# ChengZhang-98/lqer

Measured on AMD Instinct MI355X. Metric: W4A8+rank-r Linear GEMM TFLOPS-equiv, higher is better.
Workload: dtype bf16; 1 GPU; LqerLinear 4096x4096 rank32 W4A8-MXINT16 M=2048 (BASELINE configs[1]); rank=32, formats=x MXINT8/16, W MXINT4/16, A_out,B_out as x, y fp16, weights=one Linear

## Files before the change

lqer_amd/csrc/act16_fused.hip:

```cpp
#include "common.h"

namespace lqer {
namespace a16f {

constexpr int ROWS = 8, WAVES = 8, SLAB = 512, PITCH = 1040;

__host__ inline size_t lds_bytes(int rp) { return (size_t)WAVES * ROWS * PITCH + (size_t)WAVES * ROWS * rp * sizeof(float); }

typedef __attribute__((ext_vector_type(8))) __bf16 bf16v8;

#ifdef LQER_CLOCKPROBE
__device__ unsigned long long* g_a16_stamp_buf = nullptr;
#define A16_STAMP(i) asm volatile("s_memtime %0\n\ts_waitcnt lgkmcnt(0)" : "=s"(cp[i])::"memory")
#else
#define A16_STAMP(i)
#endif

template <int DT, int RT>
__global__ __launch_bounds__(512) void k_act16_fused(const void* __restrict__ x, int64_t M, int64_t K, int64_t ld, QP qx, bf16_t* __restrict__ xq,
                                                      int64_t Kp, const bf16_t* __restrict__ a_frag, QP qa, int L_aout, bf16_t* __restrict__ xaq) {
  constexpr int RP = 16 * RT;
  constexpr int HB = RT == 8 ? 2 : (RT == 4 ? 4 : 8);
  constexpr int NPART = 16 / HB;
  extern __shared__ __attribute__((aligned(16))) unsigned char smem[];
  const int lane = threadIdx.x & 63;
  const int wave = __builtin_amdgcn_readfirstlane(threadIdx.x >> 6);
  unsigned char* const wb = smem + (size_t)wave * ROWS * PITCH;
  float* const red = (float*)(smem + (size_t)WAVES * ROWS * PITCH);
  const int64_t m0 = (int64_t)blockIdx.x * ROWS;
  const int nslab = (int)((Kp + SLAB - 1) / SLAB);
  const int g = lane >> 4;
  const unsigned char* const tok = wb + (lane & 7) * PITCH + 16 * g;
  const u32x4* const fr = (const u32x4*)a_frag + lane;
  f32x4 acc[RT];
#pragma unroll
  for (int t = 0; t < RT; ++t) acc[t] = (f32x4){0.f, 0.f, 0.f, 0.f};
#ifdef LQER_CLOCKPROBE
  unsigned long long cp[8] = {0, 0, 0, 0, 0, 0, 0, 0};
  A16_STAMP(0);
#endif

  for (int s = wave; s < nslab; s += WAVES) {
    const int64_t k0 = (int64_t)s * SLAB + 8 * lane;
    const bool in_img = k0 < Kp, in_x = k0 < K;
    u32x4 raw[ROWS];
#pragma unroll
    for (int r = 0; r < ROWS; ++r)
      raw[r] = (in_x && m0 + r < M) ? *(const u32x4*)((const bf16_t*)x + (m0 + r) * ld + k0) : (u32x4){0, 0, 0, 0};
    const int st0 = s * (SLAB / 32), nst = (int)(Kp / 32);
    u32x4 fa[HB][RT], fb[HB][RT];
    auto load_part = [&](u32x4 (&f)[HB][RT], int part) {
#pragma unroll
      for (int i = 0; i < HB; ++i)
#pragma unroll
        for (int t = 0; t < RT; ++t) {
          const int st = st0 + part * HB + i;
          f[i][t] = fr[((int64_t)(st < nst ? st : 0) * RT + t) * 64];
        }
    };
    if (s == wave) A16_STAMP(1);
#pragma unroll
    for (int r = 0; r < ROWS; ++r) {
      if (r == 1 && s == wave) A16_STAMP(2);
      if (r == 2) {
        asm volatile("" ::: "memory");
        load_part(fa, 0);
        asm volatile("" ::: "memory");
      }
      if (r == 5) {
        asm volatile("" ::: "memory");
        load_part(fb, 1);
        asm volatile("" ::: "memory");
      }
      float v[8];
      const uint32_t wd[4] = {raw[r][0], raw[r][1], raw[r][2], raw[r][3]};
#pragma unroll
      for (int j = 0; j < 4; ++j) {
        if constexpr (DT == LQER_F16) {
          typedef __attribute__((ext_vector_type(2))) _Float16 h2;
          const h2 h = __builtin_bit_cast(h2, wd[j]);
          v[2 * j] = (float)h[0], v[2 * j + 1] = (float)h[1];
        } else {
          v[2 * j] = __uint_as_float(wd[j] << 16), v[2 * j + 1] = __uint_as_float(wd[j] & 0xffff0000u);
        }
      }
      float amax = 0.f;
#pragma unroll
      for (int i = 0; i < 8; ++i) amax = fmaxf(amax, fabsf(v[i]));
      amax = fmaxf(amax, __shfl_xor(amax, 1, 64));
      uint32_t w[4] = {0, 0, 0, 0};
      if (amax > 0.f) {
        const int e = block_exponent_u(amax, qx);
        if (mxint16_fast_ok(e, qx)) {
          mxint16_bf16_fast<DT != LQER_F16, 8>(v, e, qx, w);
        } else {
#pragma unroll
          for (int i = 0; i < 4; ++i) {
            const uint32_t lo = exact_bf16_bits(ldexpf(mxint_mantissa(v[2 * i], e, qx), e - qx.mbits));
            const uint32_t hi = exact_bf16_bits(ldexpf(mxint_mantissa(v[2 * i + 1], e, qx), e - qx.mbits));
            w[i] = lo | (hi << 16);
          }
        }
      }
      const u32x4 wv = {w[0], w[1], w[2], w[3]};
      if (in_img) *(u32x4*)(xq + (m0 + r) * Kp + k0) = wv;
      *(u32x4*)(wb + r * PITCH + 16 * lane) = wv;
    }
    if (s == wave) A16_STAMP(3);
    __builtin_amdgcn_fence(__ATOMIC_RELEASE, "wavefront");
    __builtin_amdgcn_wave_barrier();
    __builtin_amdgcn_fence(__ATOMIC_ACQUIRE, "wavefront");
    auto half = [&](const u32x4 (&f)[HB][RT], int t0) {
      u32x4 tk[HB];
#pragma unroll
      for (int i = 0; i < HB; ++i) tk[i] = *(const u32x4*)(tok + 64 * (t0 + i));
#pragma unroll
      for (int i = 0; i < HB; ++i)
#pragma unroll
        for (int t = 0; t < RT; ++t)
          acc[t] = __builtin_amdgcn_mfma_f32_16x16x32_bf16(__builtin_bit_cast(bf16v8, tk[i]), __builtin_bit_cast(bf16v8, f[i][t]), acc[t], 0, 0, 0);
    };
#pragma unroll
    for (int pp = 0; pp < NPART; pp += 2) {
      half(fa, pp * HB);
      if (pp + 2 < NPART) load_part(fa, pp + 2);
      half(fb, (pp + 1) * HB);
      if (pp + 3 < NPART) load_part(fb, pp + 3);
    }
    __builtin_amdgcn_fence(__ATOMIC_RELEASE, "wavefront");
    __builtin_amdgcn_wave_barrier();
#ifdef LQER_CLOCKPROBE
    if (s == wave) {
      asm volatile("" ::"v"(acc[0]));
      A16_STAMP(4);
    }
#endif
  }
  if (g < 2) {
#pragma unroll
    for (int t = 0; t < RT; ++t)
#pragma unroll
      for (int j = 0; j < 4; ++j) red[(wave * ROWS + 4 * g + j) * RP + 16 * t + (lane & 15)] = acc[t][j];
  }
  __syncthreads();
#ifdef LQER_CLOCKPROBE
  A16_STAMP(5);
  if (g_a16_stamp_buf && lane == 0) {
    unsigned long long* o = g_a16_stamp_buf + ((size_t)blockIdx.x * WAVES + wave) * 8;
    for (int i = 1; i < 6; ++i) o[i] = cp[i] - cp[0];
    unsigned long long rt;
    asm volatile("s_memrealtime %0\n\ts_waitcnt lgkmcnt(0)" : "=s"(rt)::"memory");
    o[0] = cp[0], o[6] = rt;
  }
#endif
  const int tid = threadIdx.x;
  const bool live = tid < ROWS * RP / 4;
  const int r = tid / (RP / 4), c4 = tid - r * (RP / 4);
  float4 sum = make_float4(0.f, 0.f, 0.f, 0.f);
  if (live) {
#pragma unroll
    for (int w = 0; w < WAVES; ++w) {
      const float4 v = *(const float4*)(red + (w * ROWS + r) * RP + 4 * c4);
      sum.x += v.x, sum.y += v.y, sum.z += v.z, sum.w += v.w;
    }
  }
  if (tid >= 64 * ((ROWS * RP / 4 + 63) / 64)) return;
  float bmax = fmaxf(fmaxf(fabsf(sum.x), fabsf(sum.y)), fmaxf(fabsf(sum.z), fabsf(sum.w)));
  const int G = L_aout / 4;
  for (int d = 1; d < G; d <<= 1) bmax = fmaxf(bmax, __shfl_xor(bmax, d, 64));
  if (!live || m0 + r >= M) return;
  const bool anyb = bmax > 0.f;
  const int eb = anyb ? block_exponent(bmax, qa) : 0;
  const float v[4] = {sum.x, sum.y, sum.z, sum.w};
  uint32_t w2[2];
#pragma unroll
  for (int i = 0; i < 2; ++i) {
    const float m0v = anyb ? mxint_mantissa(v[2 * i], eb, qa) : 0.f;
    const float m1v = anyb ? mxint_mantissa(v[2 * i + 1], eb, qa) : 0.f;
    w2[i] = exact_bf16_bits(ldexpf(m0v, eb - qa.mbits)) | (exact_bf16_bits(ldexpf(m1v, eb - qa.mbits)) << 16);
  }
  *(uint2*)(xaq + ((m0 + r) * RP + 4 * c4)) = make_uint2(w2[0], w2[1]);
}

__global__ __launch_bounds__(256) void k_a_b16(const bf16_t* __restrict__ limb0, int64_t Kp, int rp, bf16_t* __restrict__ out) {
  const int RT = rp / 16;
  const int64_t n_img = (int64_t)rp * Kp / 8, total = 2 * n_img;
  for (int64_t idx = (int64_t)blockIdx.x * 256 + threadIdx.x; idx < total; idx += (int64_t)gridDim.x * 256) {
    if (idx < n_img) {
      ((u32x4*)out)[idx] = ((const u32x4*)limb0)[idx];
    } else {
      const int64_t f = idx - n_img;
      const int lane = (int)(f & 63);
      const int64_t blk = f >> 6;
      const int t = (int)(blk % RT);
      const int64_t s = blk / RT;
      ((u32x4*)out)[idx] = *(const u32x4*)(limb0 + (int64_t)(16 * t + (lane & 15)) * Kp + 32 * s + 8 * (lane >> 4));
    }
  }
}

}

#ifdef LQER_CLOCKPROBE
extern "C" int lqer_debug_set_a16_stamp_buffer(void* p) { return (int)hipMemcpyToSymbol(HIP_SYMBOL(a16f::g_a16_stamp_buf), &p, sizeof(p)); }
#endif

size_t a_b16_image_bytes(int64_t K, int64_t r) { return (size_t)2 * lqer_padded_r(r) * lqer_padded_k(K) * sizeof(bf16_t); }

int a_b16_prepare_dispatch(const void* a_t_limbs, int64_t K, int64_t r, void* out, hipStream_t st) {
  const int64_t rp = lqer_padded_r(r), Kp = lqer_padded_k(K);
  if (rp % 16 != 0 || Kp % 32 != 0) {
    set_error("a_b16_prepare: padded rank %d / padded K %d", (int)rp, (int)Kp);
    return LQER_E_UNSUPPORTED;
  }
  const int64_t total = 2 * rp * Kp / 8;
  a16f::k_a_b16<<<(unsigned)((total + 255) / 256 < 4096 ? (total + 255) / 256 : 4096), 256, 0, st>>>((const bf16_t*)a_t_limbs, Kp, (int)rp, (bf16_t*)out);
  return check_launch("a_b16_prepare");
}

int act16_fused_dispatch(const void* x, int dtype, int64_t M, int64_t K, int64_t ldx, const QP& qx, bf16_t* xq, const void* a_b16, int64_t r,
                         const QP& qa, bf16_t* xaq, int tuning, hipStream_t st) {
  if (tuning & LQER_TUNE_ACT16_SPLIT) return LQER_E_UNSUPPORTED;
  const int64_t rp = lqer_padded_r(r), Kp = lqer_padded_k(K);
  if (dtype == LQER_F32 || !a_b16 || !xaq || !xq || r <= 0 || M <= 0) return LQER_E_UNSUPPORTED;
  if (!(rp == 16 || rp == 32 || rp == 64)) return LQER_E_UNSUPPORTED;
  if (qx.kind != LQER_Q_MXINT || qx.block != 16 || qx.mbits > 8) return LQER_E_UNSUPPORTED;
  if (((uintptr_t)x % 16) != 0 || ((ldx * 2) % 16) != 0 || K % 16 != 0) return LQER_E_UNSUPPORTED;
  if (qa.kind != LQER_Q_MXINT || qa.mbits > 8) return LQER_E_UNSUPPORTED;
  const int L = (qa.block <= 0 || qa.block >= rp) ? (int)rp : qa.block;
  const int G = L / 4;
  if (rp % L != 0 || L % 4 != 0 || (G & (G - 1)) != 0 || G > 64) return LQER_E_UNSUPPORTED;
  if (!(tuning & LQER_TUNE_ACT16_FUSED) && (M > LQER_ACT8_FUSED_MAX_M || M < LQER_ACT8_FUSED_MIN_M)) return LQER_E_UNSUPPORTED;
  const bf16_t* const a_frag = (const bf16_t*)a_b16 + rp * Kp;
  const unsigned grid = (unsigned)((M + a16f::ROWS - 1) / a16f::ROWS);
  const int lds = (int)a16f::lds_bytes((int)rp);
#define A16F_LAUNCH(DTv, RTv)                                                                                              \
  do {                                                                                                                     \
    static LdsLimitOnce once;                                                                                              \
    once.set((const void*)a16f::k_act16_fused<DTv, RTv>, 160 * 1024);                                                       \
    a16f::k_act16_fused<DTv, RTv><<<grid, 512, lds, st>>>(x, M, K, ldx, qx, xq, Kp, a_frag, qa, L, xaq);                     \
  } while (0)
#define A16F_DT(DTv)                     \
  switch (rp / 16) {                     \
    case 1: A16F_LAUNCH(DTv, 1); break;  \
    case 2: A16F_LAUNCH(DTv, 2); break;  \
    default: A16F_LAUNCH(DTv, 4); break; \
  }
  if (dtype == LQER_F16) {
    A16F_DT(LQER_F16)
  } else {
    A16F_DT(LQER_BF16)
  }
#undef A16F_DT
#undef A16F_LAUNCH
  return check_launch("quantize_act_xa (fused block-16 route)");
}

}
```

Before: 1057 TFLOP/s-equiv.

## Split fused act16 quantize+XA kernel across 16 waves sharing slabs

```diff
diff --git a/lqer_amd/csrc/act16_fused.hip b/lqer_amd/csrc/act16_fused.hip
--- a/lqer_amd/csrc/act16_fused.hip
+++ b/lqer_amd/csrc/act16_fused.hip
@@ -3,9 +3,9 @@
 namespace lqer {
 namespace a16f {
 
-constexpr int ROWS = 8, WAVES = 8, SLAB = 512, PITCH = 1040;
-
-__host__ inline size_t lds_bytes(int rp) { return (size_t)WAVES * ROWS * PITCH + (size_t)WAVES * ROWS * rp * sizeof(float); }
+constexpr int ROWS = 8, SLABS = 8, WAVES = 16, WROWS = 4, SLAB = 512, PITCH = 1040;
+
+__host__ inline size_t lds_bytes(int rp) { return (size_t)SLABS * ROWS * PITCH + (size_t)SLABS * ROWS * rp * sizeof(float); }
 
 typedef __attribute__((ext_vector_type(8))) __bf16 bf16v8;
 
@@ -16,141 +16,217 @@
 #define A16_STAMP(i)
 #endif
 
+__device__ __forceinline__ float pair_max(float v) {
+  return fmaxf(v, __int_as_float(__builtin_amdgcn_update_dpp(0, __float_as_int(v), 0xB1, 0xf, 0xf, true)));
+}
+
+template <int DT>
+__device__ __forceinline__ void row_values(const u32x4& raw, float (&v)[8]) {
+#pragma unroll
+  for (int i = 0; i < 4; ++i) {
+    const uint32_t wd = raw[i];
+    if constexpr (DT == LQER_F16) {
+      typedef __attribute__((ext_vector_type(2))) _Float16 h2;
+      const h2 hh = __builtin_bit_cast(h2, wd);
+      v[2 * i] = (float)hh[0], v[2 * i + 1] = (float)hh[1];
+    } else {
+      v[2 * i] = __uint_as_float(wd << 16), v[2 * i + 1] = __uint_as_float(wd & 0xffff0000u);
+    }
+  }
+}
+
+template <int DT>
+__device__ __forceinline__ u32x4 row_bits(const float (&v)[8]) {
+  u32x4 r;
+#pragma unroll
+  for (int i = 0; i < 4; ++i) {
+    if constexpr (DT == LQER_F16) r[i] = __builtin_bit_cast(uint32_t, __builtin_amdgcn_cvt_pkrtz(v[2 * i], v[2 * i + 1]));
+    else r[i] = (__float_as_uint(v[2 * i]) >> 16) | (__float_as_uint(v[2 * i + 1]) & 0xffff0000u);
+  }
+  return r;
+}
+
+template <int DT>
+__device__ __forceinline__ void quantize_rows_slow(unsigned char* rows, const QP& qx, bf16_t* img, int64_t Kp, bool in_img) {
+#pragma unroll 1
+  for (int j = 0; j < WROWS; ++j) {
+    float v[8];
+    row_values<DT>(*(const u32x4*)(rows + j * PITCH), v);
+    float amax = 0.f;
+#pragma unroll
+    for (int i = 0; i < 8; ++i) amax = fmaxf(amax, fabsf(v[i]));
+    amax = pair_max(amax);
+    uint32_t w[4] = {0, 0, 0, 0};
+    if (amax > 0.f) {
+      const int e = block_exponent_u(amax, qx);
+      if (mxint16_fast_ok(e, qx)) {
+        mxint16_bf16_fast<DT != LQER_F16, 8>(v, e, qx, w);
+      } else {
+#pragma unroll
+        for (int i = 0; i < 4; ++i) {
+          const uint32_t lo = exact_bf16_bits(ldexpf(mxint_mantissa(v[2 * i], e, qx), e - qx.mbits));
+          const uint32_t hi = exact_bf16_bits(ldexpf(mxint_mantissa(v[2 * i + 1], e, qx), e - qx.mbits));
+          w[i] = lo | (hi << 16);
+        }
+      }
+    }
+    const u32x4 wv = {w[0], w[1], w[2], w[3]};
+    if (in_img) *(u32x4*)(img + j * Kp) = wv;
+    *(u32x4*)(rows + j * PITCH) = wv;
+  }
+}
+
 template <int DT, int RT>
-__global__ __launch_bounds__(512) void k_act16_fused(const void* __restrict__ x, int64_t M, int64_t K, int64_t ld, QP qx, bf16_t* __restrict__ xq,
-                                                      int64_t Kp, const bf16_t* __restrict__ a_frag, QP qa, int L_aout, bf16_t* __restrict__ xaq) {
+__global__ __launch_bounds__(1024) void k_act16_fused(const void* __restrict__ x, int64_t M, int64_t K, int64_t ld, QP qx, bf16_t* __restrict__ xq,
+                                                       int64_t Kp, const bf16_t* __restrict__ a_frag, QP qa, int L_aout, bf16_t* __restrict__ xaq) {
   constexpr int RP = 16 * RT;
-  constexpr int HB = RT == 8 ? 2 : (RT == 4 ? 4 : 8);
+  constexpr int TW = RT >= 2 ? RT / 2 : 1;
+  constexpr int HB = TW == 2 ? 4 : 8;
   constexpr int NPART = 16 / HB;
   extern __shared__ __attribute__((aligned(16))) unsigned char smem[];
+  asm volatile("" ::"s"(x), "s"(M), "s"(K), "s"(ld), "s"(xq), "s"(Kp), "s"(a_frag), "s"(xaq), "s"(L_aout), "s"(qx.mbits), "s"(qx.emin), "s"(qx.emax),
+               "s"(qx.mmax), "s"(qx.mneg), "s"(qx.eps), "s"(qx.tiny), "s"(qa.mbits), "s"(qa.emin), "s"(qa.emax), "s"(qa.mmax), "s"(qa.mneg), "s"(qa.eps),
+               "s"(qa.tiny));
   const int lane = threadIdx.x & 63;
   const int wave = __builtin_amdgcn_readfirstlane(threadIdx.x >> 6);
-  unsigned char* const wb = smem + (size_t)wave * ROWS * PITCH;
-  float* const red = (float*)(smem + (size_t)WAVES * ROWS * PITCH);
+  const int sl = wave & (SLABS - 1), h = wave >> 3;
+  unsigned char* const sb = smem + (size_t)sl * ROWS * PITCH;
+  float* const red = (float*)(smem + (size_t)SLABS * ROWS * PITCH);
   const int64_t m0 = (int64_t)blockIdx.x * ROWS;
   const int nslab = (int)((Kp + SLAB - 1) / SLAB);
+  const int ntrip = (nslab + SLABS - 1) / SLABS;
   const int g = lane >> 4;
-  const unsigned char* const tok = wb + (lane & 7) * PITCH + 16 * g;
+  const unsigned char* const tok = sb + (lane & 7) * PITCH + 16 * g;
   const u32x4* const fr = (const u32x4*)a_frag + lane;
-  f32x4 acc[RT];
-#pragma unroll
-  for (int t = 0; t < RT; ++t) acc[t] = (f32x4){0.f, 0.f, 0.f, 0.f};
+  const int t0w = RT >= 2 ? h * TW : 0;
+  const int64_t row0 = m0 + WROWS * h;
+  const int nrow = M - row0 >= WROWS ? WROWS : (int)(M - row0);
+  const int xstep = (int)(ld * 2), qstep = (int)(Kp * 2);
+  const auto xr = __builtin_amdgcn_make_buffer_rsrc((void*)((const unsigned char*)x + row0 * ld * 2), 0, nrow > 0 ? (nrow - 1) * xstep + (int)(K * 2) : 0,
+                                                    0x00020000);
+  const auto qr = __builtin_amdgcn_make_buffer_rsrc((void*)((unsigned char*)xq + row0 * Kp * 2), 0, WROWS * qstep, 0x00020000);
+  f32x4 acc[TW];
+#pragma unroll
+  for (int t = 0; t < TW; ++t) acc[t] = (f32x4){0.f, 0.f, 0.f, 0.f};
 #ifdef LQER_CLOCKPROBE
   unsigned long long cp[8] = {0, 0, 0, 0, 0, 0, 0, 0};
   A16_STAMP(0);
 #endif
 
-  for (int s = wave; s < nslab; s += WAVES) {
-    const int64_t k0 = (int64_t)s * SLAB + 8 * lane;
-    const bool in_img = k0 < Kp, in_x = k0 < K;
-    u32x4 raw[ROWS];
-#pragma unroll
-    for (int r = 0; r < ROWS; ++r)
-      raw[r] = (in_x && m0 + r < M) ? *(const u32x4*)((const bf16_t*)x + (m0 + r) * ld + k0) : (u32x4){0, 0, 0, 0};
+  for (int it = 0; it < ntrip; ++it) {
+    const int s = it * SLABS + sl;
+    const bool live_slab = s < nslab;
     const int st0 = s * (SLAB / 32), nst = (int)(Kp / 32);
-    u32x4 fa[HB][RT], fb[HB][RT];
-    auto load_part = [&](u32x4 (&f)[HB][RT], int part) {
+    u32x4 fa[HB][TW], fb[HB][TW];
+    auto load_part = [&](u32x4 (&f)[HB][TW], int part) {
 #pragma unroll
       for (int i = 0; i < HB; ++i)
 #pragma unroll
-        for (int t = 0; t < RT; ++t) {
+        for (int t = 0; t < TW; ++t) {
           const int st = st0 + part * HB + i;
-          f[i][t] = fr[((int64_t)(st < nst ? st : 0) * RT + t) * 64];
+          f[i][t] = fr[((int64_t)(st < nst ? st : 0) * RT + t0w + t) * 64];
         }
     };
-    if (s == wave) A16_STAMP(1);
-#pragma unroll
-    for (int r = 0; r < ROWS; ++r) {
-      if (r == 1 && s == wave) A16_STAMP(2);
-      if (r == 2) {
-        asm volatile("" ::: "memory");
-        load_part(fa, 0);
-        asm volatile("" ::: "memory");
-      }
-      if (r == 5) {
-        asm volatile("" ::: "memory");
-        load_part(fb, 1);
-        asm volatile("" ::: "memory");
-      }
-      float v[8];
-      const uint32_t wd[4] = {raw[r][0], raw[r][1], raw[r][2], raw[r][3]};
-#pragma unroll
-      for (int j = 0; j < 4; ++j) {
-        if constexpr (DT == LQER_F16) {
-          typedef __attribute__((ext_vector_type(2))) _Float16 h2;
-          const h2 h = __builtin_bit_cast(h2, wd[j]);
-          v[2 * j] = (float)h[0], v[2 * j + 1] = (float)h[1];
-        } else {
-          v[2 * j] = __uint_as_float(wd[j] << 16), v[2 * j + 1] = __uint_as_float(wd[j] & 0xffff0000u);
+    if (live_slab) {
+      const int kb = s * (SLAB * 2) + 16 * lane;
+      const int xoff = kb < (int)(K * 2) ? kb : -1 - WROWS * xstep, qoff = kb < qstep ? kb : -1 - WROWS * qstep;
+      u32x4 raw[WROWS];
+#pragma unroll
+      for (int j = 0; j < WROWS; ++j) raw[j] = __builtin_amdgcn_raw_buffer_load_b128(xr, xoff + j * xstep, 0, 0);
+      load_part(fa, 0);
+      if (it == 0) A16_STAMP(1);
+      float v[WROWS][8], amax[WROWS];
+      int e[WROWS];
+      bool near = false;
+#pragma unroll
+      for (int j = 0; j < WROWS; ++j) {
+        row_values<DT>(raw[j], v[j]);
+        float a = 0.f;
+#pragma unroll
+        for (int i = 0; i < 8; ++i) a = fmaxf(a, fabsf(v[j][i]));
+        amax[j] = a = pair_max(a);
+        const uint32_t bits = __float_as_uint(a);
+        const int eb = (int)((bits >> 23) & 0xff) - 126;
+        e[j] = eb < qx.emin ? qx.emin : (eb > qx.emax ? qx.emax : eb);
+        near |= (bits & 0x7fffffu) <= 22u && a > 0.f;
+      }
+      if (__builtin_amdgcn_ballot_w64(near) != 0) {
+#pragma unroll
+        for (int j = 0; j < WROWS; ++j) e[j] = block_exponent(amax[j], qx);
+      }
+      bool slow = false;
+#pragma unroll
+      for (int j = 0; j < WROWS; ++j) slow |= amax[j] > 0.f && !mxint16_fast_ok(e[j], qx);
+      if (it == 0) A16_STAMP(2);
+      if (__builtin_amdgcn_ballot_w64(slow) == 0) {
+        uint32_t w[WROWS][4];
+#pragma unroll
+        for (int j = 0; j < WROWS; ++j) {
+          mxint16_bf16_fast<DT != LQER_F16, 8>(v[j], e[j], qx, w[j]);
+          uint32_t keep = amax[j] > 0.f ? 0xffffffffu : 0u;
+          asm("" : "+v"(keep));
+#pragma unroll
+          for (int i = 0; i < 4; ++i) w[j][i] &= keep;
         }
-      }
-      float amax = 0.f;
-#pragma unroll
-      for (int i = 0; i < 8; ++i) amax = fmaxf(amax, fabsf(v[i]));
-      amax = fmaxf(amax, __shfl_xor(amax, 1, 64));
-      uint32_t w[4] = {0, 0, 0, 0};
-      if (amax > 0.f) {
-        const int e = block_exponent_u(amax, qx);
-        if (mxint16_fast_ok(e, qx)) {
-          mxint16_bf16_fast<DT != LQER_F16, 8>(v, e, qx, w);
-        } else {
-#pragma unroll
-          for (int i = 0; i < 4; ++i) {
-            const uint32_t lo = exact_bf16_bits(ldexpf(mxint_mantissa(v[2 * i], e, qx), e - qx.mbits));
-            const uint32_t hi = exact_bf16_bits(ldexpf(mxint_mantissa(v[2 * i + 1], e, qx), e - qx.mbits));
-            w[i] = lo | (hi << 16);
-          }
+#pragma unroll
+        for (int j = 0; j < WROWS; ++j) {
+          const u32x4 wv = {w[j][0], w[j][1], w[j][2], w[j][3]};
+          __builtin_amdgcn_raw_buffer_store_b128(wv, qr, qoff + j * qstep, 0, 0);
+          *(u32x4*)(sb + (WROWS * h + j) * PITCH + 16 * lane) = wv;
         }
-      }
-      const u32x4 wv = {w[0], w[1], w[2], w[3]};
-      if (in_img) *(u32x4*)(xq + (m0 + r) * Kp + k0) = wv;
-      *(u32x4*)(wb + r * PITCH + 16 * lane) = wv;
-    }
-    if (s == wave) A16_STAMP(3);
-    __builtin_amdgcn_fence(__ATOMIC_RELEASE, "wavefront");
-    __builtin_amdgcn_wave_barrier();
-    __builtin_amdgcn_fence(__ATOMIC_ACQUIRE, "wavefront");
-    auto half = [&](const u32x4 (&f)[HB][RT], int t0) {
-      u32x4 tk[HB];
-#pragma unroll
-      for (int i = 0; i < HB; ++i) tk[i] = *(const u32x4*)(tok + 64 * (t0 + i));
-#pragma unroll
-      for (int i = 0; i < HB; ++i)
-#pragma unroll
-        for (int t = 0; t < RT; ++t)
-          acc[t] = __builtin_amdgcn_mfma_f32_16x16x32_bf16(__builtin_bit_cast(bf16v8, tk[i]), __builtin_bit_cast(bf16v8, f[i][t]), acc[t], 0, 0, 0);
-    };
-#pragma unroll
-    for (int pp = 0; pp < NPART; pp += 2) {
-      half(fa, pp * HB);
-      if (pp + 2 < NPART) load_part(fa, pp + 2);
-      half(fb, (pp + 1) * HB);
-      if (pp + 3 < NPART) load_part(fb, pp + 3);
-    }
-    __builtin_amdgcn_fence(__ATOMIC_RELEASE, "wavefront");
-    __builtin_amdgcn_wave_barrier();
-#ifdef LQER_CLOCKPROBE
-    if (s == wave) {
+      } else {
+#pragma unroll
+        for (int j = 0; j < WROWS; ++j) *(u32x4*)(sb + (WROWS * h + j) * PITCH + 16 * lane) = row_bits<DT>(v[j]);
+        quantize_rows_slow<DT>(sb + WROWS * h * PITCH + 16 * lane, qx, xq + (m0 + WROWS * h) * Kp + (int64_t)s * SLAB + 8 * lane, Kp,
+                               (int64_t)s * SLAB + 8 * lane < Kp);
+      }
+      load_part(fb, 1);
+      if (it == 0) A16_STAMP(3);
+    }
+    __syncthreads();
+    if (it == 0) A16_STAMP(4);
+    if (live_slab) {
+      auto half = [&](const u32x4 (&f)[HB][TW], int t0) {
+        u32x4 tk[HB];
+#pragma unroll
+        for (int i = 0; i < HB; ++i) tk[i] = *(const u32x4*)(tok + 64 * (t0 + i));
+#pragma unroll
+        for (int i = 0; i < HB; ++i)
+#pragma unroll
+          for (int t = 0; t < TW; ++t)
+            acc[t] = __builtin_amdgcn_mfma_f32_16x16x32_bf16(__builtin_bit_cast(bf16v8, tk[i]), __builtin_bit_cast(bf16v8, f[i][t]), acc[t], 0, 0, 0);
+      };
+#pragma unroll
+      for (int pp = 0; pp < NPART; pp += 2) {
+        half(fa, pp * HB);
+        if (pp + 2 < NPART) load_part(fa, pp + 2);
+        half(fb, (pp + 1) * HB);
+        if (pp + 3 < NPART) load_part(fb, pp + 3);
+      }
+    }
+#ifdef LQER_CLOCKPROBE
+    if (it == 0) {
       asm volatile("" ::"v"(acc[0]));
-      A16_STAMP(4);
-    }
-#endif
-  }
-  if (g < 2) {
-#pragma unroll
-    for (int t = 0; t < RT; ++t)
-#pragma unroll
-      for (int j = 0; j < 4; ++j) red[(wave * ROWS + 4 * g + j) * RP + 16 * t + (lane & 15)] = acc[t][j];
+      A16_STAMP(5);
+    }
+#endif
+    if (it + 1 < ntrip) __syncthreads();
+  }
+  if (g < 2 && (RT >= 2 || h == 0)) {
+#pragma unroll
+    for (int t = 0; t < TW; ++t)
+#pragma unroll
+      for (int j = 0; j < 4; ++j) red[(sl * ROWS + 4 * g + j) * RP + 16 * (t0w + t) + (lane & 15)] = acc[t][j];
   }
   __syncthreads();
 #ifdef LQER_CLOCKPROBE
-  A16_STAMP(5);
+  A16_STAMP(6);
   if (g_a16_stamp_buf && lane == 0) {
     unsigned long long* o = g_a16_stamp_buf + ((size_t)blockIdx.x * WAVES + wave) * 8;
-    for (int i = 1; i < 6; ++i) o[i] = cp[i] - cp[0];
+    for (int i = 1; i < 7; ++i) o[i] = cp[i] - cp[0];
     unsigned long long rt;
     asm volatile("s_memrealtime %0\n\ts_waitcnt lgkmcnt(0)" : "=s"(rt)::"memory");
-    o[0] = cp[0], o[6] = rt;
+    o[0] = cp[0], o[7] = rt;
   }
 #endif
   const int tid = threadIdx.x;
@@ -159,7 +235,7 @@
   float4 sum = make_float4(0.f, 0.f, 0.f, 0.f);
   if (live) {
 #pragma unroll
-    for (int w = 0; w < WAVES; ++w) {
+    for (int w = 0; w < SLABS; ++w) {
       const float4 v = *(const float4*)(red + (w * ROWS + r) * RP + 4 * c4);
       sum.x += v.x, sum.y += v.y, sum.z += v.z, sum.w += v.w;
     }
@@ -167,7 +243,15 @@
   if (tid >= 64 * ((ROWS * RP / 4 + 63) / 64)) return;
   float bmax = fmaxf(fmaxf(fabsf(sum.x), fabsf(sum.y)), fmaxf(fabsf(sum.z), fabsf(sum.w)));
   const int G = L_aout / 4;
-  for (int d = 1; d < G; d <<= 1) bmax = fmaxf(bmax, __shfl_xor(bmax, d, 64));
+  float o;
+  o = __int_as_float(__builtin_amdgcn_update_dpp(0, __float_as_int(bmax), 0xB1, 0xf, 0xf, true));
+  bmax = G > 1 ? fmaxf(bmax, o) : bmax;
+  o = __int_as_float(__builtin_amdgcn_update_dpp(0, __float_as_int(bmax), 0x4E, 0xf, 0xf, true));
+  bmax = G > 2 ? fmaxf(bmax, o) : bmax;
+  o = __int_as_float(__builtin_amdgcn_update_dpp(0, __float_as_int(bmax), 0x141, 0xf, 0xf, true));
+  bmax = G > 4 ? fmaxf(bmax, o) : bmax;
+  o = __int_as_float(__builtin_amdgcn_update_dpp(0, __float_as_int(bmax), 0x140, 0xf, 0xf, true));
+  bmax = G > 8 ? fmaxf(bmax, o) : bmax;
   if (!live || m0 + r >= M) return;
   const bool anyb = bmax > 0.f;
   const int eb = anyb ? block_exponent(bmax, qa) : 0;
@@ -229,7 +313,7 @@
   if (qa.kind != LQER_Q_MXINT || qa.mbits > 8) return LQER_E_UNSUPPORTED;
   const int L = (qa.block <= 0 || qa.block >= rp) ? (int)rp : qa.block;
   const int G = L / 4;
-  if (rp % L != 0 || L % 4 != 0 || (G & (G - 1)) != 0 || G > 64) return LQER_E_UNSUPPORTED;
+  if (rp % L != 0 || L % 4 != 0 || (G & (G - 1)) != 0 || G > 16) return LQER_E_UNSUPPORTED;
   if (!(tuning & LQER_TUNE_ACT16_FUSED) && (M > LQER_ACT8_FUSED_MAX_M || M < LQER_ACT8_FUSED_MIN_M)) return LQER_E_UNSUPPORTED;
   const bf16_t* const a_frag = (const bf16_t*)a_b16 + rp * Kp;
   const unsigned grid = (unsigned)((M + a16f::ROWS - 1) / a16f::ROWS);
@@ -238,7 +322,7 @@
   do {                                                                                                                     \
     static LdsLimitOnce once;                                                                                              \
     once.set((const void*)a16f::k_act16_fused<DTv, RTv>, 160 * 1024);                                                       \
-    a16f::k_act16_fused<DTv, RTv><<<grid, 512, lds, st>>>(x, M, K, ldx, qx, xq, Kp, a_frag, qa, L, xaq);                     \
+    a16f::k_act16_fused<DTv, RTv><<<grid, 64 * a16f::WAVES, lds, st>>>(x, M, K, ldx, qx, xq, Kp, a_frag, qa, L, xaq);                     \
   } while (0)
 #define A16F_DT(DTv)                     \
   switch (rp / 16) {                     \
```

Measured after the change: 1063 TFLOP/s-equiv (median of 4 runs). About the same (+0.6%).
